# QualityMinds/cistgcn

Hardware: AMD Instinct MI355X
Metric: sequences/sec (fwd+bwd) H3.6M 22-joint 50->25 (higher is better)
Workload: dtype f32; 1 GPU; cistgcn64_b256_t50_v22; C=64, per_gpu_batch=256, global_batch=256, T_in=50, T_out=25, V=22, parallelism=dp1, graph=True, graph_branches=True, capture_kept=median, mixed_batches=False

## Files before the change

### cistgcn_amd/_lib.py

```python
import ctypes
import os
from ctypes import POINTER, c_double, c_float, c_int, c_int32, c_longlong, c_uint, c_ulonglong, c_void_p

HERE = os.path.dirname(os.path.abspath(__file__))
LIB_PATH = os.path.join(HERE, "libcistgcn_hip.so")

_handle = None
STAT_REPLICAS = 16
ALPHA_SLOTS = 64
_host_pointers_ok = False


class View4(ctypes.Structure):
    _fields_ = [("n", c_longlong * 4), ("s", c_longlong * 4)]


class NormAct(ctypes.Structure):
    _fields_ = [
        ("x", c_void_p), ("xv", View4),
        ("y", c_void_p), ("yv", View4),
        ("pre", c_void_p),
        ("add", c_void_p), ("av", View4),
        ("add_post", c_int),
        ("bn_mode", c_int),
# ... 101 lines not shown
                ("dx", c_void_p), ("dgamma", c_void_p), ("dbeta", c_void_p)]


class GatePath(ctypes.Structure):
    _fields_ = [("z", c_void_p), ("stats", c_void_p), ("stats_ld", c_longlong),
                ("bn2", TailBN), ("alpha2", c_void_p), ("Wl", c_void_p), ("bn3", TailBN), ("alpha3", c_void_p), ("W2", c_void_p),
                ("salt2", c_uint), ("salt3", c_uint), ("y", c_void_p), ("w", c_void_p), ("tap2", c_void_p), ("tap3", c_void_p),
                ("dw", c_void_p), ("dz", c_void_p), ("dstats", c_void_p), ("dWl", c_void_p), ("dW2", c_void_p),
                ("dgamma2", c_void_p), ("dbeta2", c_void_p), ("dalpha2", c_void_p), ("dgamma3", c_void_p), ("dbeta3", c_void_p), ("dalpha3", c_void_p),
                ("scratch", c_void_p), ("red", c_void_p)]


class GateHead(ctypes.Structure):
    _fields_ = [("B", c_int), ("C", c_int), ("S", c_int), ("train", c_int), ("n", c_int), ("pad", c_int),
                ("drop_p", c_float), ("pad2", c_int), ("seed", c_void_p), ("p", GatePath * 2)]


class CtxHeads(ctypes.Structure):
    _fields_ = [("B", c_int), ("P", c_int), ("C", c_int), ("train", c_int), ("x", c_void_p), ("xstats", c_void_p),
                ("w", c_void_p * 2), ("bn", TailBN * 2), ("alpha", c_void_p * 2),
                ("y", c_void_p * 2), ("arg", c_void_p), ("xsave", c_void_p), ("tap", c_void_p * 2),
                ("dy", c_void_p * 2), ("red", c_void_p), ("dx", c_void_p),
                ("dw", c_void_p * 2), ("dgamma", c_void_p * 2), ("dbeta", c_void_p * 2), ("dalpha", c_void_p * 2)]


class AttackStep(ctypes.Structure):
    _fields_ = [("B", c_int), ("T", c_int), ("V", c_int), ("mode", c_int), ("iterations", c_int), ("patience", c_int),
                ("epsilon", c_float), ("mu", c_float),
                ("x0", c_void_p), ("x", c_void_p), ("grad", c_void_p), ("g", c_void_p), ("mask", c_void_p), ("loss", c_void_p),
                ("best", c_void_p), ("stall", c_void_p), ("active", c_void_p), ("w", c_void_p), ("queries", c_void_p), ("n_active", c_void_p),
# ... 64 lines not shown
    "cg_collapse_sums_ws_floats": [c_int, c_int],
    "cg_fpn_conv_fwd": [POINTER(FpnConv), P],
    "cg_fpn_conv_bwd": [POINTER(FpnConv), P],
    "cg_fpn_conv_supported": [c_int, c_int, c_int, c_int, c_int],
    "cg_fpn_conv_ws_floats": [c_int, c_int, c_int, c_int],
    "cg_pointwise_maps_fwd": [POINTER(PwMaps), P],
    "cg_pointwise_maps_bwd": [POINTER(PwMaps), P],
    "cg_pointwise_maps_ws_floats": [c_int],
    "cg_block_input_fwd": [POINTER(BlockInput), P],
    "cg_block_input_bwd": [POINTER(BlockInput), P],
    "cg_block_input_supported": [c_int, c_int, c_int, c_int],
    "cg_gate_head_fwd": [POINTER(GateHead), P],
    "cg_gate_head_bwd": [POINTER(GateHead), P],
    "cg_gate_head_supported": [c_int, c_int, c_int],
    "cg_gate_head_scratch_floats": [c_int, c_int, c_int],
    "cg_context_heads_fwd": [POINTER(CtxHeads), P],
    "cg_context_heads_bwd": [POINTER(CtxHeads), P],
    "cg_context_heads_red_doubles": [c_int],
    "cg_map2adj_tail_fwd": [POINTER(AdjTail), c_int, c_int, P],
    "cg_map2adj_tail_bwd": [POINTER(AdjTail), c_int, c_int, P],
    "cg_map2adj_tail_ws_floats": [c_int],
    "cg_map2adj_tail_part_floats": [c_int, c_int, c_int],
    "cg_map2adj_tail_red_doubles": [c_int],
    "cg_augment_sequences": [P, P, P, P, P, P, P, P, P, P, c_int, c_int, c_int, c_int, P],
    "cg_map2adj_tail_geometry": [c_int, c_int, c_int, POINTER(c_int)],
    "cg_dstd_tail_geometry": [c_int, c_int, c_int, c_int, POINTER(c_int)],
    "cg_pointwise_maps_geometry": [c_int, c_int, c_int, c_int, POINTER(c_int), c_int, POINTER(c_int)],
    "cg_collapse_geometry": [c_int, c_int, c_int, c_int, c_int, c_int, POINTER(c_int)],
    "cg_fpn_conv_geometry": [c_int, c_int, c_int, c_int, c_int, POINTER(c_int)],
    "cg_stgcn_domain_geometry": [c_int, c_int, c_int, c_int, c_int, c_int, c_int, c_int, POINTER(c_int)],
# ... 47 lines not shown
```

### cistgcn_amd/models/CISTGCN/CISTGCN.py

```python
import torch
import torch.nn as nn

from ... import ops
from ..layers.SE import SELayer1d, SELayer2d


class Stage(nn.Module):

    def __init__(self, **slots):
        super().__init__()
        for k, m in slots.items():
            self.add_module(k.lstrip("s"), m)

    def __getitem__(self, i):
        return self._modules[str(i)]


def _conv(cin, cout, k=1, bias=False, **kw):
    return nn.Conv2d(cin, cout, k, bias=bias, **kw)


def _init_small(root, gain, convs):
    for m in root.modules():
        if isinstance(m, nn.Linear):
# ... 155 lines not shown
        p = arch.model_params
        self.clipping = p.clipping
        self.n_input, self.n_output, self.n_joints = p.input_n, p.output_n, p.joints
        self.n_txcnn_layers = p.n_txcnn_layers
        self.txc_kernel_size = [p.txc_kernel_size] * 2
        self.input_gcn, self.output_gcn = p.input_gcn, p.output_gcn
        self.reduction, self.hidden_dim = p.reduction, p.hidden_dim
        self.dropout = float(learn.dropout)
        self.in_ch = 10
        self.fused_domain = True
        self.staged = True
        self.fused_tail = True
        self.fused_adj = True
        self.fused_maps = True
        self.fused_defer = True
        self.stack_min_elements = 1 << 21
        widths = [self.in_ch] + list(p.input_gcn.model_complexity) + [self.in_ch]
        widths_o = [3] + list(p.output_gcn.model_complexity)
        T, V, To = self.n_input, self.n_joints, self.n_output

        self.st_gcnns = nn.ModuleList()
        self.txcnns = nn.ModuleList()
        self.se = nn.ModuleList()
        self.in_conv = nn.ModuleList()
        self.context_layer = nn.ModuleList()
        self.trans = nn.ModuleList()
        for i in range(len(widths) - 1):
            self.st_gcnns.append(DSTDBlock(widths[i], widths[i + 1], p.input_gcn.interpretable[i], T, V, self.reduction))
        self.context_layer = ContextLayer(self.hidden_dim, To, V, self.reduction)
        self.txcnns.append(FPN(T, To, p.txc_kernel_size))
# ... 160 lines not shown
            xa = list(ops.fanout(xn0, n_alias))
        x_stats, xn, x_dom = xa[0], xa[1], xa[2:4]
        k = 4
        x_maps = x_gates = None
        if stacked:
            x_maps, k = xa[4], 5
        if rows_gate:
            x_gates, k = xa[k], k + 1
        x_resmaps = []
        if res_groups:
            x_resmaps, k = xa[k:k + len(res_groups)], k + len(res_groups)
        x_res = xa[k:k + 2] if not has_res else None
        x_bres = xa[-1] if not has_bres else None
        if not fused_in:
            stats_s, stats_t = ops.fanout(ops.dstd_stats(x_stats), 2)
        gate_rows = None
        if gates:
            O = cs.out_channels
            w2 = ops.cat_channels([cs.weight.view(1, O, -1), ct.weight.view(1, O, -1)]).view(2 * O, cs.in_channels, xn.shape[2])
            if x_gates is not None:
                gate_rows = ops.collapse_rows(x_gates, w2)[0]
                items = []
            else:
                items = [(("och,bchw->bow", w2, xn, None, None, None), None)]
        else:
            items = [_rows_item(xn, cs, tr), _rows_item(xn, ct, tr)]
        if not stacked:
            for a in maps:
                items += [_pw_item(xn, a.time_compress[0], tr), _pw_item(xn, a.joint_compress[0], tr)]
        if res_groups is None:
            items += [_pw_item(xn, c, tr) for c in res_convs]
        o = _run_items(items) if items else []
        if gates:
            yg = gate_rows if gate_rows is not None else o.pop(0)[0]
            o = [(g.unsqueeze(2), None) for g in ops.split_channels(yg, (O, O))] + o
        towers_done, tower_tr = None, None
# ... 40 lines not shown
                o = o + ro
        gs, gt, tc = o[0], o[1], o[2:6]
        calls = [dict(x=gs, bn=m.conv_s[1], drop=True, prelu=m.conv_s[3]), dict(x=gt, bn=m.conv_t[1], drop=True, prelu=m.conv_t[3])]
        if towers_done is None:
            for i, a in enumerate(maps):
                calls += [dict(x=tc[2 * i], bn=a.time_compress[1], prelu=a.time_compress[2]),
                          dict(x=tc[2 * i + 1], bn=a.joint_compress[1], prelu=a.joint_compress[2])]
        k = 6
        n_tower_calls = len(calls) - 2
        if res_done is None:
            if has_res:
                calls += [dict(x=o[k + i], bn=d.residual[1]) for i, d in enumerate(doms)]
                k += 2
            if has_bres:
                calls.append(dict(x=o[k], bn=m.residual[1]))
        if towers_done is None:
            r = self._na_many(calls)
        else:
            r = self._na_many(calls[:2])
            self._site += 4
            r = r + towers_done + (self._na_many(calls[2 + n_tower_calls:]) if len(calls) > 2 + n_tower_calls else [])
        if res_done is not None:
            self._site += len(res_done)
            r = r + res_done
        gs, gt, t1 = r[0], r[1], r[2:6]
        res = r[6:8] if has_res else x_res
        bres = r[-1] if has_bres else x_bres
        items = [_cols_item(gs, m.conv_s[4], tr), _cols_item(gt, m.conv_t[4], tr)]
        rows3, cols3 = {}, {}
        for i, a in enumerate(maps):
            c3 = a.time_compress[3]
            x3 = t1[2 * i][0] if isinstance(t1[2 * i], tuple) else t1[2 * i]
            w3 = c3.weight.view(c3.out_channels, c3.in_channels, -1)
            if big and c3.bias is None and ops.collapse_rows_ok(x3, w3):
                y3, st3 = ops.collapse_rows(x3, w3, tr, transform=tower_tr[2 * i] if tower_tr else None)
                rows3[i] = (y3.unsqueeze(2), st3)
            else:
                assert tower_tr is None, "a deferred tower map needs its collapsing kernel"
                items.append(_rows_item(t1[2 * i], c3, tr))
            c4 = a.joint_compress[3]
            x4 = t1[2 * i + 1][0] if isinstance(t1[2 * i + 1], tuple) else t1[2 * i + 1]
            w4 = c4.weight.view(c4.out_channels, c4.in_channels, -1)
            if big and c4.bias is None and ops.collapse_cols_ok(x4, w4):
                y4, st4 = ops.collapse_cols(x4, w4, tr, transform=tower_tr[2 * i + 1] if tower_tr else None)
                cols3[i] = (y4.unsqueeze(3), st4)
            else:
                assert tower_tr is None, "a deferred tower map needs its collapsing kernel"
                items.append(_cols_item(t1[2 * i + 1], c4, tr))
        if tower_tr and self.act_trace is not None:
            tp_ = [b_ for a_ in maps for b_ in (a_.time_compress[2], a_.joint_compress[2])]
            for mod, tr_ in zip(tp_, tower_tr):
                self.act_trace[mod] = (tr_["tap"].detach(), None)
        o = _run_items(items)
        if rows3 or cols3:
            rest, o = o[2:], o[:2]
            for i in range(len(maps)):
                o.append(rows3[i] if i in rows3 else rest.pop(0))
                o.append(cols3[i] if i in cols3 else rest.pop(0))
        Cg = m.conv_s[4].out_channels
        gate_fused = (o[0][0].shape[1] == Cg and o[0][0].numel() == B * Cg and
                      ops.gate_head_ok(B, Cg, stats_s.shape[1], (m.conv_s[7], m.conv_t[7], m.map_s[3], m.map_t[3])))
        tower_calls = []
        for i, a in enumerate(maps):
            tower_calls += [dict(x=o[2 + 2 * i], bn=a.time_compress[4], drop=True), dict(x=o[3 + 2 * i], bn=a.joint_compress[4], drop=True)]
        if gate_fused:
            s2 = (self._site + 1, self._site + 2)
            self._site += 2
            r = [None, None] + self._na_many(tower_calls)
            s3 = (self._site + 1, self._site + 2)
            self._site += 2
            if self.drop_trace is not None:
                self.drop_trace[m.conv_s[5]], self.drop_trace[m.conv_t[5]], self.drop_trace[m.map_s[1]], self.drop_trace[m.map_t[1]] = s2[0], s2[1], s3[0], s3[1]
            taps = [] if self.act_trace is not None else None
            m.w1, m.w2 = ops.gate_head([o[0][0].view(B, Cg), o[1][0].view(B, Cg)], [stats_s, stats_t], [m.conv_s, m.conv_t], [m.map_s, m.map_t], tr,
                                       drop_p=self.dropout, salts=((s2[0], s3[0]), (s2[1], s3[1])), taps=taps)
            if taps is not None:
                self.act_trace[m.conv_s[7]], self.act_trace[m.map_s[3]] = (taps[0], None), (taps[1], None)
                self.act_trace[m.conv_t[7]], self.act_trace[m.map_t[3]] = (taps[2], None), (taps[3], None)
            items, g = [], None
        else:
            calls = [dict(x=o[0], bn=m.conv_s[5], drop=True, prelu=m.conv_s[7]), dict(x=o[1], bn=m.conv_t[5], drop=True, prelu=m.conv_t[7])]
            r = self._na_many(calls + tower_calls)
            hs = ops.cat_channels([r[0].view(B, -1), stats_s])
            ht = ops.cat_channels([r[1].view(B, -1), stats_t])
            items = [_lin_item(hs, m.map_s[0], tr), _lin_item(ht, m.map_t[0], tr)]
        for i, a in enumerate(maps):
            items += [_pw_item(r[2 + 2 * i], a.time_compress[6], False), _pw_item(r[3 + 2 * i], a.joint_compress[6], False)]
        o = _run_items(items)
        if gate_fused:
            o = [None, None] + o
        else:
            g = self._na_many([dict(x=o[0], bn=m.map_s[1], drop=True, prelu=m.map_s[3]), dict(x=o[1], bn=m.map_t[1], drop=True, prelu=m.map_t[3])])
        seeds = []
        for i, d in enumerate(doms):
            q, s = o[2 + 2 * i][0].view(B, T, V), o[3 + 2 * i][0].view(B, V, T)
            seeds.append((0 if d.domain == "space" else 1, s, q))
        if self.fused_adj and T <= 64 and V <= 64:
            if not gate_fused:
                o = _run_items([_lin_item(g[0], m.map_s[4], False), _lin_item(g[1], m.map_t[4], False)])
                m.w1, m.w2 = o[0][0], o[1][0]
            self._site += 2
            if self.drop_trace is not None:
                self.drop_trace[maps[0].expansor[1]], self.drop_trace[maps[1].expansor[1]] = self._site - 1, self._site
            taps = [] if self.act_trace is not None else None
            adj = ops.map2adj_tail(seeds, [a.expansor for a in maps], tr, drop_p=self.dropout, salts=(self._site - 1, self._site), taps=taps)
            adj = [(a, None) for a in adj]
            if taps is not None:
                for a, tap in zip(maps, taps):
                    self.act_trace[a.expansor[3]] = (tap, None)
        else:
            if T <= 64 and V <= 64:
                oo = ops.rank1_adj(seeds)
# ... 150 lines not shown
```

### cistgcn_amd/ops.py

```python
import ctypes
import os

import numpy as np
import torch

from . import _lib
from ._lib import NormAct, View4

_vp = ctypes.c_void_p


def _ptr(t):
    return _vp(t.data_ptr()) if t is not None else None


def _stream(t):
    if t.is_cuda:
        return _vp(torch.cuda.current_stream(t.device).cuda_stream)
    if not _lib._host_pointers_ok:
        raise RuntimeError("cistgcn_amd operators run on MI355X only: got a %s tensor (no CPU path exists)" % t.device)
    return None


def _chk(t, name="tensor"):
# ... 1935 lines not shown
        _lib.call("cg_gate_head_bwd", ctypes.byref(t), _stream(ts[0]))
        del keep
        return (None, None) + tuple(g if ctx.needs_input_grad[2 + k] else None for k, g in enumerate(grads))


def gate_head(zs, stats, convs, maps, train, drop_p=0.0, salts=((0, 0), (0, 0)), taps=None):
    n = len(zs)
    cfg = {"train": bool(train), "drop_p": float(drop_p), "salts": tuple((int(a), int(b)) for a, b in salts),
           "bn2": tuple(c[5] for c in convs), "bn3": tuple(m[1] for m in maps), "taps": taps}
    ts = []
    for z, st, c, m in zip(zs, stats, convs, maps):
        ts += [z, st, c[5].weight, c[5].bias, c[7].weight, m[0].weight, m[1].weight, m[1].bias, m[3].weight, m[4].weight]
    return list(_GateHead.apply(cfg, n, *ts))


def context_heads_ok(x, hidden):
    return x.dim() == 4 and x.shape[1] == 1 and x.is_contiguous() and hidden <= 64 and x.shape[2] * x.shape[3] <= 16384


class _ContextHeads(torch.autograd.Function):

    @staticmethod
    def _block(x, ts, bns, saves, train):
        B, _, H, W = x.shape
        t = _lib.CtxHeads()
        t.B, t.P, t.C, t.train = B, H * W, ts[0].numel(), 1 if train else 0
        t.x = x.data_ptr()
        for h in range(2):
            w, gamma, beta, alpha = ts[4 * h:4 * h + 4]
            t.w[h], t.alpha[h] = w.data_ptr(), alpha.data_ptr()
# ... 438 lines not shown
```

### include/cistgcn_hip.h

```cpp
#ifndef CISTGCN_HIP_H
#define CISTGCN_HIP_H
#include <stdint.h>
#ifdef __cplusplus
extern "C" {
#endif

#define CG_STAT_REPLICAS 16
#define CG_ALPHA_SLOTS 64

typedef struct CgView4 {
  long long n[4];
  long long s[4];
} CgView4;

int cg_contract(const float* A, const float* X, float* Y, const float* bias, double* stats, const int32_t* tables,
                int G, int M, int N, int K, int splitk, int a_kfast, int x_kfast,
                long long y_dense_numel, void* stream);

typedef struct CgContractDesc {
  const float* A; const float* X; float* Y; const float* bias; double* stats; const int32_t* tab;
  int G, M, N, K, splitk, kchunk , a_kfast, x_kfast;
  int accumulate;
  int x_vec;
  int stat_ch;
// ... 219 lines not shown
  float* dWl; float* dW2;
  float* dgamma2; float* dbeta2; float* dalpha2; float* dgamma3; float* dbeta3; float* dalpha3;
  float* scratch;
  double* red;
} CgGatePath;
typedef struct CgGateHead {
  int B, C, S, train, n, pad;
  float drop_p; int pad2; const unsigned long long* seed;
  CgGatePath p[2];
} CgGateHead;
int cg_gate_head_fwd(const CgGateHead* t, void* stream);
int cg_gate_head_bwd(const CgGateHead* t, void* stream);
int cg_gate_head_supported(int B, int C, int S);
long long cg_gate_head_scratch_floats(int B, int C, int S);

typedef struct CgCtxHeads {
  int B, P, C, train;
  const float* x;
  const double* xstats;
  const float* w[2]; CgTailBN bn[2]; const float* alpha[2];
  float* y[2];
  int32_t* arg;
  float* xsave;
  float* tap[2];
  const float* dy[2];
  double* red;
  float* dx;
  float* dw[2]; float* dgamma[2]; float* dbeta[2]; float* dalpha[2];
} CgCtxHeads;
int cg_context_heads_fwd(const CgCtxHeads* t, void* stream);
// ... 64 lines not shown
```

Baseline: 14750 sequences/sec.

## Fuse block mid-stage BN/PReLU/dropout/linear maps into batched multi-item kernel

Adds a block_mid HIP kernel family that, for up to six items per launch, applies batch norm from the producer's channel sums, PReLU and dropout, then a full linear map or a pointwise map, with matching two-kernel backward producing dx, dW, dgamma, dbeta and dalpha. The model's map stage routes through it instead of separate per-item launches and intermediate tensors. The aim is fewer launches and less global memory traffic for the normalized activations. In exchange it adds per-slice partial weight-gradient buffers and a second reduction pass, and it only runs for supported shapes.

```diff
diff --git a/cistgcn_amd/_lib.py b/cistgcn_amd/_lib.py
--- a/cistgcn_amd/_lib.py
+++ b/cistgcn_amd/_lib.py
@@ -139,6 +139,19 @@
 class GateHead(ctypes.Structure):
     _fields_ = [("B", c_int), ("C", c_int), ("S", c_int), ("train", c_int), ("n", c_int), ("pad", c_int),
                 ("drop_p", c_float), ("pad2", c_int), ("seed", c_void_p), ("p", GatePath * 2)]
+
+
+class MidItem(ctypes.Structure):
+    _fields_ = [("kind", c_int), ("C", c_int), ("L", c_int), ("O", c_int), ("sb_", c_int), ("ns_", c_int),
+                ("x", c_void_p), ("x_ld", c_longlong), ("bn", TailBN), ("stats_ld", c_longlong), ("alpha", c_void_p), ("W", c_void_p),
+                ("salt", c_uint), ("pad", c_int), ("y", c_void_p), ("tap", c_void_p),
+                ("dy", c_void_p), ("dx", c_void_p), ("dW", c_void_p), ("dgamma", c_void_p), ("dbeta", c_void_p), ("dalpha", c_void_p),
+                ("g", c_void_p), ("part", c_void_p), ("wpart", c_void_p)]
+
+
+class BlockMid(ctypes.Structure):
+    _fields_ = [("B", c_int), ("train", c_int), ("n", c_int), ("pad", c_int),
+                ("drop_p", c_float), ("pad2", c_int), ("seed", c_void_p), ("it", MidItem * 6)]
 
 
 class CtxHeads(ctypes.Structure):
@@ -233,6 +246,10 @@
     "cg_gate_head_bwd": [POINTER(GateHead), P],
     "cg_gate_head_supported": [c_int, c_int, c_int],
     "cg_gate_head_scratch_floats": [c_int, c_int, c_int],
+    "cg_block_mid_fwd": [POINTER(BlockMid), P],
+    "cg_block_mid_bwd": [POINTER(BlockMid), P],
+    "cg_block_mid_supported": [c_int, c_int, c_int, c_int, c_int],
+    "cg_block_mid_geometry": [c_int, c_int, c_int, c_int, c_int, POINTER(c_int)],
     "cg_context_heads_fwd": [POINTER(CtxHeads), P],
     "cg_context_heads_bwd": [POINTER(CtxHeads), P],
     "cg_context_heads_red_doubles": [c_int],
diff --git a/cistgcn_amd/csrc/block_mid.h b/cistgcn_amd/csrc/block_mid.h
--- /dev/null
+++ b/cistgcn_amd/csrc/block_mid.h
@@ -0,0 +1,27 @@
+#pragma once
+#include "dstd_tail.h"
+
+#define CG_MID_MAXN 6
+#define CG_MID_MAXD 64
+struct CgMidItem {
+  int kind, C, L, O;
+  int sb_, ns_;
+  const float* x; long long x_ld;
+  CgTailBN bn; long long stats_ld;
+  const float* alpha;
+  const float* W;
+  unsigned int salt; int pad;
+  float* y;
+  float* tap;
+  const float* dy;
+  float* dx;
+  float* dW; float* dgamma; float* dbeta; float* dalpha;
+  float* g;
+  double* part;
+  float* wpart;
+};
+struct CgBlockMid {
+  int B, train, n, pad;
+  float drop_p; int pad2; const unsigned long long* seed;
+  CgMidItem it[CG_MID_MAXN];
+};
diff --git a/cistgcn_amd/csrc/block_mid.hip b/cistgcn_amd/csrc/block_mid.hip
--- /dev/null
+++ b/cistgcn_amd/csrc/block_mid.hip
@@ -0,0 +1,402 @@
+#include "cg_common.h"
+#include "cg_phase.h"
+#include "block_mid.h"
+
+HIP_DYNAMIC_SHARED(unsigned char, cg_dyn_lds)
+
+#define CG_MID_THREADS 1024
+#define CG_MID_KSTEPS 4
+#define CG_MID_OSTEPS 8
+#define CG_MID_WAVES (CG_MID_THREADS / CG_WAVE)
+#define CG_MID_SB 8
+#define CG_MID_FULL_FLOATS 8192
+#define CG_MID_PW_FLOATS 4096
+
+static inline int cg_mid_pad4(int n) { return (n + 3) & ~3; }
+static inline int cg_mid_sb(int kind, int C, int L, int O) {
+  const int per = kind == 0 ? C * L : (C > O ? C : O) * L;
+  int sb = (kind == 0 ? CG_MID_FULL_FLOATS : CG_MID_PW_FLOATS) / per;
+  return sb < 1 ? 1 : (sb > CG_MID_SB ? CG_MID_SB : sb);
+}
+
+__device__ __forceinline__ void cg_mid_aff(const CgMidItem& it, int c, double cnt, int train, bool backward, bool owner, float* k) {
+  const CgTailBN& bn = it.bn;
+  const int C = it.C;
+  float mean, rstd;
+  if (backward) { mean = bn.save[c]; rstd = bn.save[C + c]; }
+  else if (train) {
+    double s1 = 0.0, s2 = 0.0;
+    for (int r = 0; r < CG_STAT_REPLICAS; ++r) { s1 += bn.stats[((long long)r * it.stats_ld + c) * 2]; s2 += bn.stats[((long long)r * it.stats_ld + c) * 2 + 1]; }
+    const double m = s1 / cnt;
+    double var = s2 / cnt - m * m;
+    if (var < 0.0) var = 0.0;
+    mean = (float)m;
+    rstd = (float)(1.0 / sqrt(var + (double)bn.eps));
+    if (owner && bn.running_mean) {
+      const double unb = cnt > 1.0 ? var * cnt / (cnt - 1.0) : var;
+      bn.running_mean[c] = (1.f - bn.momentum) * bn.running_mean[c] + bn.momentum * (float)m;
+      bn.running_var[c] = (1.f - bn.momentum) * bn.running_var[c] + bn.momentum * (float)unb;
+      if (c == 0 && bn.num_batches_tracked) *bn.num_batches_tracked += 1;
+    }
+  } else {
+    mean = bn.running_mean[c];
+    rstd = 1.0f / sqrtf(bn.running_var[c] + bn.eps);
+  }
+  if (!backward && owner) { bn.save[c] = mean; bn.save[C + c] = rstd; }
+  k[0] = mean; k[1] = rstd; k[2] = bn.gamma[c] * rstd; k[3] = bn.beta[c];
+}
+
+__device__ __forceinline__ float cg_mid_u(const CgBlockMid& t, const CgMidItem& it, const float (*sAff)[4], unsigned long long seed, bool drop,
+                                          int b, int r, int K, float& keep, float& xv) {
+  const int c = r / it.L;
+  xv = it.x[(long long)b * it.x_ld + r];
+  keep = drop ? cg_drop_scale(t.drop_p, seed, it.salt, (unsigned long long)b * K + r) : 1.f;
+  return ((xv - sAff[c][0]) * sAff[c][2] + sAff[c][3]) * keep;
+}
+
+__device__ __forceinline__ void cg_mid_stage_h(const CgBlockMid& t, const CgMidItem& it, const float (*sAff)[4], float* sH, int b0, int nb, bool tap) {
+  const int K = it.C * it.L;
+  const bool drop = t.train && t.drop_p > 0.f;
+  const unsigned long long seed = drop ? *t.seed : 0ull;
+  for (int e = threadIdx.x; e < it.sb_ * K; e += CG_MID_THREADS) {
+    const int b = e / K, r = e - b * K;
+    float h = 0.f;
+    if (b < nb) {
+      float keep, xv;
+      const float u = cg_mid_u(t, it, sAff, seed, drop, b0 + b, r, K, keep, xv);
+      h = it.alpha ? (u > 0.f ? u : it.alpha[0] * u) : u;
+      if (tap && it.tap) it.tap[(long long)(b0 + b) * K + r] = h;
+    }
+    sH[e] = h;
+  }
+}
+
+__global__ __launch_bounds__(CG_MID_THREADS) void cg_block_mid_fwd_kernel(CgBlockMid t) {
+  const CgMidItem& it = t.it[blockIdx.y];
+  if ((int)blockIdx.x >= it.ns_) return;
+  const int C = it.C, L = it.L, O = it.O, K = C * L, sb = it.sb_;
+  const int tid = threadIdx.x, lane = tid & (CG_WAVE - 1), wave = tid / CG_WAVE;
+  const int b0 = (int)blockIdx.x * sb, nb = min(sb, t.B - b0);
+  __shared__ float sAff[CG_MID_MAXD][4];
+  __shared__ double sRed[CG_MID_WAVES][4 * CG_MID_SB][4];
+  float* sH = reinterpret_cast<float*>(cg_dyn_lds);
+  float* sW = sH + ((sb * K + 3) & ~3);
+  const int OP = (O + 3) & ~3;
+  if (tid < C) cg_mid_aff(it, tid, (double)t.B * L, t.train, false, blockIdx.x == 0, sAff[tid]);
+  if (it.kind == 1)
+    for (int e = tid; e < C * OP; e += CG_MID_THREADS) { const int c = e / OP, o = e - c * OP; sW[e] = o < O ? it.W[o * C + c] : 0.f; }
+  __syncthreads();
+  cg_mid_stage_h(t, it, sAff, sH, b0, nb, true);
+  __syncthreads();
+  if (it.kind == 1) {
+    const int OG = OP >> 2, total = nb * OG * L;
+    for (int idx = tid; idx < total; idx += CG_MID_THREADS) {
+      const int l = idx % L, r = idx / L, og = r % OG, b = r / OG;
+      const float* h = sH + b * K + l;
+      const float* w = sW + 4 * og;
+      float acc[4] = {0.f, 0.f, 0.f, 0.f};
+      for (int c = 0; c < C; ++c) {
+        const float hv = h[c * L];
+        const float4 wv = *reinterpret_cast<const float4*>(w + c * OP);
+        acc[0] = fmaf(wv.x, hv, acc[0]); acc[1] = fmaf(wv.y, hv, acc[1]); acc[2] = fmaf(wv.z, hv, acc[2]); acc[3] = fmaf(wv.w, hv, acc[3]);
+      }
+#pragma unroll
+      for (int j = 0; j < 4; ++j)
+        if (4 * og + j < O) it.y[((long long)(b0 + b) * O + 4 * og + j) * L + l] = acc[j];
+    }
+    return;
+  }
+  const int OG = (O + 3) >> 2, iters = (OG + CG_MID_WAVES - 1) / CG_MID_WAVES;
+  for (int i = 0; i < iters; ++i) {
+    const int og = i * CG_MID_WAVES + wave;
+    float acc[4][CG_MID_SB];
+#pragma unroll
+    for (int j = 0; j < 4; ++j)
+#pragma unroll
+      for (int b = 0; b < CG_MID_SB; ++b) acc[j][b] = 0.f;
+    if (og < OG) {
+      const float* w[4];
+#pragma unroll
+      for (int j = 0; j < 4; ++j) w[j] = it.W + (long long)min(4 * og + j, O - 1) * K;
+      for (int k0 = lane; k0 < K; k0 += CG_MID_KSTEPS * CG_WAVE) {
+        float wv[CG_MID_KSTEPS][4];
+#pragma unroll
+        for (int s = 0; s < CG_MID_KSTEPS; ++s)
+#pragma unroll
+          for (int j = 0; j < 4; ++j) wv[s][j] = k0 + s * CG_WAVE < K ? w[j][k0 + s * CG_WAVE] : 0.f;
+#pragma unroll
+        for (int s = 0; s < CG_MID_KSTEPS; ++s) {
+          const int k = k0 + s * CG_WAVE;
+          if (k < K) {
+#pragma unroll
+            for (int b = 0; b < CG_MID_SB; ++b)
+              if (b < sb) {
+                const float hv = sH[b * K + k];
+#pragma unroll
+                for (int j = 0; j < 4; ++j) acc[j][b] = fmaf(wv[s][j], hv, acc[j][b]);
+              }
+          }
+        }
+      }
+    }
+#pragma unroll
+    for (int j = 0; j < 4; ++j)
+#pragma unroll
+      for (int b = 0; b < CG_MID_SB; ++b) {
+        const double v = cg_row16_sum((double)acc[j][b]);
+        if ((lane & 15) == 0) sRed[wave][j * CG_MID_SB + b][lane >> 4] = v;
+      }
+    __syncthreads();
+    if (tid < CG_MID_WAVES * 4 * CG_MID_SB) {
+      const int w2 = tid / (4 * CG_MID_SB), q = tid - w2 * (4 * CG_MID_SB), j = q / CG_MID_SB, b = q - j * CG_MID_SB;
+      const int o = 4 * (i * CG_MID_WAVES + w2) + j;
+      if (o < O && b < nb) it.y[(long long)(b0 + b) * O + o] = (float)((sRed[w2][q][0] + sRed[w2][q][1]) + (sRed[w2][q][2] + sRed[w2][q][3]));
+    }
+    __syncthreads();
+  }
+}
+
+__global__ __launch_bounds__(CG_MID_THREADS) void cg_block_mid_bwd1_kernel(CgBlockMid t) {
+  const CgMidItem& it = t.it[blockIdx.y];
+  if ((int)blockIdx.x >= it.ns_) return;
+  const int C = it.C, L = it.L, O = it.O, K = C * L, sb = it.sb_;
+  const int tid = threadIdx.x, lane = tid & (CG_WAVE - 1), wave = tid / CG_WAVE;
+  const int slice = (int)blockIdx.x, b0 = slice * sb, nb = min(sb, t.B - b0);
+  __shared__ float sAff[CG_MID_MAXD][4];
+  __shared__ double sRedD[CG_MID_WAVES];
+  const int HK = (sb * K + 3) & ~3;
+  float* sH = reinterpret_cast<float*>(cg_dyn_lds);
+  float* sG = sH + HK;
+  float* sDy = sG + HK;
+  const int CP = (C + 3) & ~3;
+  float* sW = sDy + (it.kind == 0 ? O * CG_MID_SB : ((sb * O * L + 3) & ~3));
+  if (tid < C) cg_mid_aff(it, tid, 0.0, t.train, true, false, sAff[tid]);
+  if (it.kind == 0) {
+    for (int e = tid; e < O * CG_MID_SB; e += CG_MID_THREADS) {
+      const int o = e / CG_MID_SB, b = e - o * CG_MID_SB;
+      sDy[e] = b < nb ? it.dy[(long long)(b0 + b) * O + o] : 0.f;
+    }
+  } else {
+    for (int e = tid; e < O * CP; e += CG_MID_THREADS) { const int o = e / CP, c = e - o * CP; sW[e] = c < C ? it.W[o * C + c] : 0.f; }
+    for (int e = tid; e < nb * O * L; e += CG_MID_THREADS) sDy[e] = it.dy[(long long)b0 * O * L + e];
+  }
+  __syncthreads();
+  cg_mid_stage_h(t, it, sAff, sH, b0, nb, false);
+  __syncthreads();
+  if (it.kind == 0) {
+    float* wp = it.wpart + (long long)slice * O * K;
+    for (int k = tid; k < K; k += CG_MID_THREADS) {
+      float hv[CG_MID_SB], dh[CG_MID_SB];
+#pragma unroll
+      for (int b = 0; b < CG_MID_SB; ++b) { hv[b] = b < sb ? sH[b * K + k] : 0.f; dh[b] = 0.f; }
+      for (int o0 = 0; o0 < O; o0 += CG_MID_OSTEPS) {
+        float wv[CG_MID_OSTEPS];
+#pragma unroll
+        for (int s = 0; s < CG_MID_OSTEPS; ++s) wv[s] = o0 + s < O ? it.W[(long long)(o0 + s) * K + k] : 0.f;
+#pragma unroll
+        for (int s = 0; s < CG_MID_OSTEPS; ++s) {
+          const int o = o0 + s;
+          if (o < O) {
+            const float4 d0 = *reinterpret_cast<const float4*>(sDy + o * CG_MID_SB), d1 = *reinterpret_cast<const float4*>(sDy + o * CG_MID_SB + 4);
+            const float d[CG_MID_SB] = {d0.x, d0.y, d0.z, d0.w, d1.x, d1.y, d1.z, d1.w};
+            float a = 0.f;
+#pragma unroll
+            for (int b = 0; b < CG_MID_SB; ++b) { dh[b] = fmaf(wv[s], d[b], dh[b]); a = fmaf(d[b], hv[b], a); }
+            wp[(long long)o * K + k] = a;
+          }
+        }
+      }
+#pragma unroll
+      for (int b = 0; b < CG_MID_SB; ++b) if (b < sb) sG[b * K + k] = dh[b];
+    }
+  } else {
+    float* wp = it.wpart + (long long)slice * O * C;
+    const int OG = (O + 3) >> 2;
+    for (int e = tid; e < OG * C; e += CG_MID_THREADS) {
+      const int og = e / C, c = e - og * C;
+      int oo[4];
+#pragma unroll
+      for (int j = 0; j < 4; ++j) oo[j] = min(4 * og + j, O - 1);
+      float a[4] = {0.f, 0.f, 0.f, 0.f};
+      for (int b = 0; b < nb; ++b) {
+        const float* h = sH + b * K + c * L;
+        const float* d = sDy + b * O * L;
+        float ab[4] = {0.f, 0.f, 0.f, 0.f};
+        for (int l = 0; l < L; ++l) {
+          const float hv = h[l];
+#pragma unroll
+          for (int j = 0; j < 4; ++j) ab[j] = fmaf(d[oo[j] * L + l], hv, ab[j]);
+        }
+#pragma unroll
+        for (int j = 0; j < 4; ++j) a[j] += ab[j];
+      }
+#pragma unroll
+      for (int j = 0; j < 4; ++j) if (4 * og + j < O) wp[(4 * og + j) * C + c] = a[j];
+    }
+    const int CG = CP >> 2, total = nb * CG * L;
+    for (int idx = tid; idx < total; idx += CG_MID_THREADS) {
+      const int l = idx % L, r = idx / L, cg = r % CG, b = r / CG;
+      const float* d = sDy + b * O * L + l;
+      float acc[4] = {0.f, 0.f, 0.f, 0.f};
+      for (int o = 0; o < O; ++o) {
+        const float dv = d[o * L];
+        const float4 wv = *reinterpret_cast<const float4*>(sW + o * CP + 4 * cg);
+        acc[0] = fmaf(wv.x, dv, acc[0]); acc[1] = fmaf(wv.y, dv, acc[1]); acc[2] = fmaf(wv.z, dv, acc[2]); acc[3] = fmaf(wv.w, dv, acc[3]);
+      }
+#pragma unroll
+      for (int j = 0; j < 4; ++j) if (4 * cg + j < C) sG[b * K + (4 * cg + j) * L + l] = acc[j];
+    }
+  }
+  __syncthreads();
+  const bool drop = t.train && t.drop_p > 0.f;
+  const unsigned long long seed = drop ? *t.seed : 0ull;
+  const float alpha = it.alpha ? it.alpha[0] : 1.f;
+  double SA = 0.0;
+  for (int e = tid; e < nb * K; e += CG_MID_THREADS) {
+    const int b = e / K, r = e - b * K;
+    float keep, xv;
+    const float u = cg_mid_u(t, it, sAff, seed, drop, b0 + b, r, K, keep, xv);
+    const float dh = sG[e];
+    const bool neg = it.alpha && !(u > 0.f);
+    if (neg) SA += (double)dh * (double)u;
+    const float g = (neg ? alpha * dh : dh) * keep;
+    sG[e] = g;
+    it.g[(long long)(b0 + b) * K + r] = g;
+  }
+  __syncthreads();
+  double* part = it.part + (long long)slice * (2 * C + 1);
+  for (int c = wave; c < C; c += CG_MID_WAVES) {
+    double s1 = 0.0, s2 = 0.0;
+    const float mean = sAff[c][0], rstd = sAff[c][1];
+    for (int i = lane; i < nb * L; i += CG_WAVE) {
+      const int b = i / L, l = i - b * L;
+      const double v = (double)sG[b * K + c * L + l];
+      s1 += v;
+      s2 += v * (double)((it.x[(long long)(b0 + b) * it.x_ld + c * L + l] - mean) * rstd);
+    }
+    s1 = cg_wave_sum(s1); s2 = cg_wave_sum(s2);
+    if (lane == 0) { part[c] = s1; part[C + c] = s2; }
+  }
+  SA = cg_block_sum(SA, sRedD);
+  if (tid == 0) part[2 * C] = SA;
+}
+
+__global__ __launch_bounds__(CG_MID_THREADS) void cg_block_mid_bwd2_kernel(CgBlockMid t) {
+  const CgMidItem& it = t.it[blockIdx.y];
+  if ((int)blockIdx.x >= it.ns_) return;
+  const int C = it.C, L = it.L, O = it.O, K = C * L, sb = it.sb_, ns = it.ns_, nv = 2 * C + 1;
+  const int tid = threadIdx.x, lane = tid & (CG_WAVE - 1), wave = tid / CG_WAVE;
+  const int slice = (int)blockIdx.x, b0 = slice * sb, nb = min(sb, t.B - b0);
+  __shared__ float sAff[CG_MID_MAXD][4];
+  __shared__ double sP[CG_MID_WAVES][2 * CG_MID_MAXD + 1];
+  __shared__ float sM[CG_MID_MAXD][2];
+  if (tid < C) cg_mid_aff(it, tid, 0.0, t.train, true, false, sAff[tid]);
+  for (int v = lane; v < nv; v += CG_WAVE) {
+    double s = 0.0;
+    for (int sl = wave; sl < ns; sl += CG_MID_WAVES) s += it.part[(long long)sl * nv + v];
+    sP[wave][v] = s;
+  }
+  __syncthreads();
+  if (tid < C) {
+    double S1 = 0.0, S2 = 0.0;
+    for (int w = 0; w < CG_MID_WAVES; ++w) { S1 += sP[w][tid]; S2 += sP[w][C + tid]; }
+    const double cnt = (double)t.B * L;
+    sM[tid][0] = t.train ? (float)(S1 / cnt) : 0.f; sM[tid][1] = t.train ? (float)(S2 / cnt) : 0.f;
+    if (slice == 0) { it.dgamma[tid] = (float)S2; it.dbeta[tid] = (float)S1; }
+  }
+  if (tid == 0 && slice == 0 && it.dalpha) {
+    double SA = 0.0;
+    for (int w = 0; w < CG_MID_WAVES; ++w) SA += sP[w][2 * C];
+    it.dalpha[0] = (float)SA;
+  }
+  __syncthreads();
+  for (int e = tid; e < nb * K; e += CG_MID_THREADS) {
+    const int b = e / K, r = e - b * K, c = r / L;
+    const long long idx = (long long)(b0 + b) * K + r;
+    const float xv = it.x[(long long)(b0 + b) * it.x_ld + r];
+    it.dx[idx] = sAff[c][2] * (it.g[idx] - sM[c][0] - (xv - sAff[c][0]) * sAff[c][1] * sM[c][1]);
+  }
+  const long long NW = (long long)O * (it.kind == 0 ? K : C), chunk = (NW + ns - 1) / ns;
+  const long long e1 = min(NW, (slice + 1) * chunk);
+  for (long long e = slice * chunk + tid; e < e1; e += CG_MID_THREADS) {
+    double a = 0.0;
+    for (int sl = 0; sl < ns; ++sl) a += (double)it.wpart[sl * NW + e];
+    it.dW[e] = (float)a;
+  }
+}
+
+static size_t cg_mid_lds_fwd(int kind, int C, int L, int O) {
+  const int sb = cg_mid_sb(kind, C, L, O);
+  return ((size_t)cg_mid_pad4(sb * C * L) + (kind == 1 ? (size_t)C * cg_mid_pad4(O) : 0)) * sizeof(float);
+}
+static size_t cg_mid_lds_bwd(int kind, int C, int L, int O) {
+  const int sb = cg_mid_sb(kind, C, L, O);
+  size_t f = (size_t)2 * cg_mid_pad4(sb * C * L);
+  f += kind == 0 ? (size_t)O * CG_MID_SB : (size_t)cg_mid_pad4(sb * O * L) + (size_t)O * cg_mid_pad4(C);
+  return f * sizeof(float);
+}
+
+extern "C" int cg_block_mid_supported(int B, int kind, int C, int L, int O) {
+  if (B <= 0 || kind < 0 || kind > 1 || C <= 0 || L <= 0 || O <= 0 || C > CG_MID_MAXD || L > CG_MID_MAXD || O > CG_MID_MAXD) return 0;
+  const int sb = cg_mid_sb(kind, C, L, O);
+  const long long ns = ((long long)B + sb - 1) / sb;
+  return (ns <= 65535 && ns * O * C * (kind == 0 ? L : 1) < (1ll << 31)) ? 1 : 0;
+}
+
+extern "C" int cg_block_mid_geometry(int B, int kind, int C, int L, int O, int* out) {
+  if (!out || !cg_block_mid_supported(B, kind, C, L, O)) return CG_ESHAPE;
+  const int sb = cg_mid_sb(kind, C, L, O), ns = (B + sb - 1) / sb;
+  out[0] = sb; out[1] = ns;
+  out[2] = (int)cg_mid_lds_fwd(kind, C, L, O); out[3] = (int)cg_mid_lds_bwd(kind, C, L, O);
+  out[4] = ns * (2 * C + 1);
+  out[5] = ns * O * C * (kind == 0 ? L : 1);
+  out[6] = kind == 0 ? (((O + 3) >> 2) + CG_MID_WAVES - 1) / CG_MID_WAVES : 0;
+  out[7] = kind == 0 ? (C * L + CG_MID_THREADS - 1) / CG_MID_THREADS : 0;
+  return CG_OK;
+}
+
+static int cg_mid_prepare(const CgBlockMid* t, bool bwd, CgBlockMid& a, int& slices, size_t& lds) {
+  if (!t || t->n < 1 || t->n > CG_MID_MAXN || t->B <= 0) return CG_EARG;
+  if (t->drop_p < 0.f || t->drop_p >= 1.f) return CG_EARG;
+  if (t->train && t->drop_p > 0.f && !t->seed) return CG_EARG;
+  a = *t;
+  slices = 0; lds = 0;
+  for (int i = 0; i < t->n; ++i) {
+    CgMidItem& p = a.it[i];
+    if (!cg_block_mid_supported(t->B, p.kind, p.C, p.L, p.O)) return CG_ESHAPE;
+    if (t->train && (long long)t->B * p.L < 2) return CG_ESHAPE;
+    if (!p.x || p.x_ld < (long long)p.C * p.L || !p.W || !p.bn.gamma || !p.bn.beta || !p.bn.save) return CG_EARG;
+    if (!bwd && (!p.y || (t->train ? (!p.bn.stats || p.stats_ld < p.C) : (!p.bn.running_mean || !p.bn.running_var)))) return CG_EARG;
+    if (bwd && (!p.dy || !p.dx || !p.dW || !p.dgamma || !p.dbeta || (p.alpha && !p.dalpha) || !p.g || !p.part || !p.wpart)) return CG_EARG;
+    p.sb_ = cg_mid_sb(p.kind, p.C, p.L, p.O);
+    p.ns_ = (t->B + p.sb_ - 1) / p.sb_;
+    if (p.ns_ > slices) slices = p.ns_;
+    const size_t l = bwd ? cg_mid_lds_bwd(p.kind, p.C, p.L, p.O) : cg_mid_lds_fwd(p.kind, p.C, p.L, p.O);
+    if (l > lds) lds = l;
+  }
+  return CG_OK;
+}
+
+extern "C" int cg_block_mid_fwd(const CgBlockMid* t, void* stream_) {
+  CgBlockMid a;
+  int slices; size_t lds;
+  int st = cg_mid_prepare(t, false, a, slices, lds);
+  if (st != CG_OK) return st;
+  if (lds > CG_LDS_DEFAULT && cg_lds_limit((const void*)cg_block_mid_fwd_kernel, lds) != hipSuccess) return CG_ESHAPE;
+  hipLaunchKernelGGL(cg_block_mid_fwd_kernel, dim3((unsigned)slices, (unsigned)a.n), dim3(CG_MID_THREADS), lds, (hipStream_t)stream_, a);
+  return cg_launch_status();
+}
+
+extern "C" int cg_block_mid_bwd(const CgBlockMid* t, void* stream_) {
+  CgBlockMid a;
+  int slices; size_t lds;
+  int st = cg_mid_prepare(t, true, a, slices, lds);
+  if (st != CG_OK) return st;
+  if (lds > CG_LDS_DEFAULT && cg_lds_limit((const void*)cg_block_mid_bwd1_kernel, lds) != hipSuccess) return CG_ESHAPE;
+  const dim3 grid((unsigned)slices, (unsigned)a.n), block(CG_MID_THREADS);
+  hipLaunchKernelGGL(cg_block_mid_bwd1_kernel, grid, block, lds, (hipStream_t)stream_, a);
+  st = cg_launch_status();
+  if (st != CG_OK) return st;
+  hipLaunchKernelGGL(cg_block_mid_bwd2_kernel, grid, block, 0, (hipStream_t)stream_, a);
+  return cg_launch_status();
+}
diff --git a/cistgcn_amd/models/CISTGCN/CISTGCN.py b/cistgcn_amd/models/CISTGCN/CISTGCN.py
--- a/cistgcn_amd/models/CISTGCN/CISTGCN.py
+++ b/cistgcn_amd/models/CISTGCN/CISTGCN.py
@@ -193,6 +193,7 @@
         self.fused_adj = True
         self.fused_maps = True
         self.fused_defer = True
+        self.fused_mid = True
         self.stack_min_elements = 1 << 21
         widths = [self.in_ch] + list(p.input_gcn.model_complexity) + [self.in_ch]
         widths_o = [3] + list(p.output_gcn.model_complexity)
@@ -383,12 +384,19 @@
         x_bres = xa[-1] if not has_bres else None
         if not fused_in:
             stats_s, stats_t = ops.fanout(ops.dstd_stats(x_stats), 2)
-        gate_rows = None
+        gate_rows = gate_sums = None
+        adj_fused = self.fused_adj and T <= 64 and V <= 64
+        mid_on = self.fused_mid and big and adj_fused
+        g4s, g4t = m.conv_s[4], m.conv_t[4]
+        mid_g = (mid_on and gates and x_gates is not None and g4s.bias is None and g4t.bias is None
+                 and tuple(g4s.kernel_size) == (1, V) and tuple(g4t.kernel_size) == (1, V) and g4s.out_channels == g4t.out_channels
+                 and ops.gate_head_ok(B, g4s.out_channels, 2 + 2 * T, (m.conv_s[7], m.conv_t[7], m.map_s[3], m.map_t[3]))
+                 and ops.block_mid_ok(B, [(0, cs.out_channels, V, g4s.out_channels, m.conv_s[3]), (0, cs.out_channels, V, g4t.out_channels, m.conv_t[3])]))
         if gates:
             O = cs.out_channels
             w2 = ops.cat_channels([cs.weight.view(1, O, -1), ct.weight.view(1, O, -1)]).view(2 * O, cs.in_channels, xn.shape[2])
             if x_gates is not None:
-                gate_rows = ops.collapse_rows(x_gates, w2)[0]
+                gate_rows, gate_sums = ops.collapse_rows(x_gates, w2, mid_g and tr)
                 items = []
             else:
                 items = [(("och,bchw->bow", w2, xn, None, None, None), None)]
@@ -459,10 +467,16 @@
                 k += 2
             if has_bres:
                 calls.append(dict(x=o[k], bn=m.residual[1]))
+        mid_x = mid_salts = None
+        if mid_g:
+            mid_x, mid_salts = [gs[0].squeeze(2), gt[0].squeeze(2)], (self._site + 1, self._site + 2)
+            self._site += 2
+            if self.drop_trace is not None:
+                self.drop_trace[m.conv_s[1]], self.drop_trace[m.conv_t[1]] = mid_salts
         if towers_done is None:
-            r = self._na_many(calls)
-        else:
-            r = self._na_many(calls[:2])
+            r = [None, None] + (self._na_many(calls[2:]) if len(calls) > 2 else []) if mid_g else self._na_many(calls)
+        else:
+            r = [None, None] if mid_g else self._na_many(calls[:2])
             self._site += 4
             r = r + towers_done + (self._na_many(calls[2 + n_tower_calls:]) if len(calls) > 2 + n_tower_calls else [])
         if res_done is not None:
@@ -471,7 +485,7 @@
         gs, gt, t1 = r[0], r[1], r[2:6]
         res = r[6:8] if has_res else x_res
         bres = r[-1] if has_bres else x_bres
-        items = [_cols_item(gs, m.conv_s[4], tr), _cols_item(gt, m.conv_t[4], tr)]
+        items = [] if mid_g else [_cols_item(gs, m.conv_s[4], tr), _cols_item(gt, m.conv_t[4], tr)]
         rows3, cols3 = {}, {}
         for i, a in enumerate(maps):
             c3 = a.time_compress[3]
@@ -496,26 +510,57 @@
             tp_ = [b_ for a_ in maps for b_ in (a_.time_compress[2], a_.joint_compress[2])]
             for mod, tr_ in zip(tp_, tower_tr):
                 self.act_trace[mod] = (tr_["tap"].detach(), None)
-        o = _run_items(items)
+        o = ([None, None] if mid_g else []) + (_run_items(items) if items else [])
         if rows3 or cols3:
             rest, o = o[2:], o[:2]
             for i in range(len(maps)):
                 o.append(rows3[i] if i in rows3 else rest.pop(0))
                 o.append(cols3[i] if i in cols3 else rest.pop(0))
         Cg = m.conv_s[4].out_channels
-        gate_fused = (o[0][0].shape[1] == Cg and o[0][0].numel() == B * Cg and
-                      ops.gate_head_ok(B, Cg, stats_s.shape[1], (m.conv_s[7], m.conv_t[7], m.map_s[3], m.map_t[3])))
+        gate_fused = mid_g or (o[0][0].shape[1] == Cg and o[0][0].numel() == B * Cg and
+                               ops.gate_head_ok(B, Cg, stats_s.shape[1], (m.conv_s[7], m.conv_t[7], m.map_s[3], m.map_t[3])))
         tower_calls = []
         for i, a in enumerate(maps):
             tower_calls += [dict(x=o[2 + 2 * i], bn=a.time_compress[4], drop=True), dict(x=o[3 + 2 * i], bn=a.joint_compress[4], drop=True)]
+        tower_mid = [(a.time_compress, a.joint_compress)[k] for a in maps for k in (0, 1)]
+        mid_t = (mid_on and gate_fused and len(rows3) == len(maps) and len(cols3) == len(maps) and all(c[6].bias is None for c in tower_mid)
+                 and ops.block_mid_ok(B, [(1, o[2 + k][0].shape[1], o[2 + k][0].numel() // (B * o[2 + k][0].shape[1]), c[6].out_channels, None)
+                                          for k, c in enumerate(tower_mid)]))
         if gate_fused:
             s2 = (self._site + 1, self._site + 2)
             self._site += 2
-            r = [None, None] + self._na_many(tower_calls)
+            if mid_t:
+                tower_salts = tuple(self._site + 1 + k for k in range(len(tower_mid)))
+                self._site += len(tower_mid)
+                if self.drop_trace is not None:
+                    for c, salt in zip(tower_mid, tower_salts):
+                        self.drop_trace[c[4]] = salt
+                r = [None] * (2 + len(tower_mid))
+            else:
+                r = [None, None] + self._na_many(tower_calls)
             s3 = (self._site + 1, self._site + 2)
             self._site += 2
             if self.drop_trace is not None:
                 self.drop_trace[m.conv_s[5]], self.drop_trace[m.conv_t[5]], self.drop_trace[m.map_s[1]], self.drop_trace[m.map_t[1]] = s2[0], s2[1], s3[0], s3[1]
+            mid_out = []
+            if mid_g or mid_t:
+                mitems = []
+                if mid_g:
+                    for i, cv in enumerate((m.conv_s, m.conv_t)):
+                        mitems.append(dict(kind=0, x=mid_x[i], bn=cv[1], prelu=cv[3], weight=cv[4].weight.view(Cg, -1, V), salt=mid_salts[i],
+                                           stats=(gate_sums, i * mid_x[i].shape[1], 2 * mid_x[i].shape[1]) if tr else None))
+                if mid_t:
+                    for k, c in enumerate(tower_mid):
+                        y, st = o[2 + k]
+                        mitems.append(dict(kind=1, x=y.view(B, y.shape[1], -1), bn=c[4], prelu=None, weight=c[6].weight.view(c[6].out_channels, y.shape[1]),
+                                           salt=tower_salts[k], stats=(st, 0, y.shape[1]) if tr else None))
+                mtaps = [] if self.act_trace is not None else None
+                mid_out = ops.block_mid(mitems, tr, drop_p=self.dropout, taps=mtaps)
+                if mid_g:
+                    o[0], o[1] = (mid_out[0], None), (mid_out[1], None)
+                    mid_out = mid_out[2:]
+                    if mtaps is not None:
+                        self.act_trace[m.conv_s[3]], self.act_trace[m.conv_t[3]] = (mtaps[0].unsqueeze(2), None), (mtaps[1].unsqueeze(2), None)
             taps = [] if self.act_trace is not None else None
             m.w1, m.w2 = ops.gate_head([o[0][0].view(B, Cg), o[1][0].view(B, Cg)], [stats_s, stats_t], [m.conv_s, m.conv_t], [m.map_s, m.map_t], tr,
                                        drop_p=self.dropout, salts=((s2[0], s3[0]), (s2[1], s3[1])), taps=taps)
@@ -529,9 +574,12 @@
             hs = ops.cat_channels([r[0].view(B, -1), stats_s])
             ht = ops.cat_channels([r[1].view(B, -1), stats_t])
             items = [_lin_item(hs, m.map_s[0], tr), _lin_item(ht, m.map_t[0], tr)]
-        for i, a in enumerate(maps):
-            items += [_pw_item(r[2 + 2 * i], a.time_compress[6], False), _pw_item(r[3 + 2 * i], a.joint_compress[6], False)]
-        o = _run_items(items)
+        if mid_t:
+            o = [(y, None) for y in mid_out]
+        else:
+            for i, a in enumerate(maps):
+                items += [_pw_item(r[2 + 2 * i], a.time_compress[6], False), _pw_item(r[3 + 2 * i], a.joint_compress[6], False)]
+            o = _run_items(items)
         if gate_fused:
             o = [None, None] + o
         else:
@@ -540,7 +588,7 @@
         for i, d in enumerate(doms):
             q, s = o[2 + 2 * i][0].view(B, T, V), o[3 + 2 * i][0].view(B, V, T)
             seeds.append((0 if d.domain == "space" else 1, s, q))
-        if self.fused_adj and T <= 64 and V <= 64:
+        if adj_fused:
             if not gate_fused:
                 o = _run_items([_lin_item(g[0], m.map_s[4], False), _lin_item(g[1], m.map_t[4], False)])
                 m.w1, m.w2 = o[0][0], o[1][0]
diff --git a/cistgcn_amd/ops.py b/cistgcn_amd/ops.py
--- a/cistgcn_amd/ops.py
+++ b/cistgcn_amd/ops.py
@@ -1973,6 +1973,127 @@
     return list(_GateHead.apply(cfg, n, *ts))
 
 
+def _mid_geometry(B, kind, C, L, O):
+    out = (ctypes.c_int * 8)()
+    _lib.check(_lib.lib().cg_block_mid_geometry(B, kind, C, L, O, out), "cg_block_mid_geometry")
+    return list(out)
+
+
+def block_mid_ok(B, items):
+    return 1 <= len(items) <= 6 and all(bool(_lib.lib().cg_block_mid_supported(B, k, C, L, O)) and (p is None or p.weight.numel() == 1)
+                                        for k, C, L, O, p in items)
+
+
+class _BlockMid(torch.autograd.Function):
+
+    @staticmethod
+    def _block(cfg, ts, saves, train, dev):
+        items = cfg["items"]
+        t = _lib.BlockMid()
+        t.B, t.train, t.n = ts[0].shape[0], 1 if train else 0, len(items)
+        p = float(cfg.get("drop_p", 0.0)) if train else 0.0
+        t.drop_p = p
+        if p > 0.0:
+            t.seed = seed_state(dev).data_ptr()
+        for i, it in enumerate(items):
+            x, _, _, a, w = ts[5 * i:5 * i + 5]
+            q = t.it[i]
+            q.kind, q.C, q.L, q.O = it["kind"], x.shape[1], x.shape[2], w.shape[0]
+            q.x, q.x_ld = x.data_ptr(), x.stride(0)
+            _tail_bn(q.bn, it["bn"], None, saves[i], train)
+            st = it.get("stats")
+            if train and st is not None:
+                q.bn.stats, q.stats_ld = st[0].data_ptr() + 16 * st[1], st[2]
+            q.alpha, q.W, q.salt = _ptr(a), w.data_ptr(), it["salt"]
+        return t, p
+
+    @staticmethod
+    def forward(ctx, cfg, *ts):
+        ctx.set_materialize_grads(False)
+        items = cfg["items"]
+        dev, f32, train = ts[0].device, torch.float32, bool(cfg["train"])
+        B = ts[0].shape[0]
+        ts = list(ts)
+        for i, it in enumerate(items):
+            x, w = ts[5 * i], ts[5 * i + 4]
+            _chk(x)
+            C, L = x.shape[1], x.shape[2]
+            if x.dim() != 3 or (L > 1 and x.stride(2) != 1) or (C > 1 and x.stride(1) != L) or x.stride(0) < C * L:
+                raise ValueError("block_mid expects (B,C,L) inputs with dense samples")
+            if w.numel() != w.shape[0] * C * (L if it["kind"] == 0 else 1):
+                raise ValueError("block_mid: weight %s does not fit input %s" % (tuple(w.shape), tuple(x.shape)))
+            if not w.is_contiguous():
+                ts[5 * i + 4] = _copy(w)
+            if train and it.get("stats") is None:
+                raise ValueError("block_mid needs the producer's channel sums in train mode")
+            if train and B * L < 2:
+                raise ValueError("Expected more than 1 value per channel when training, got input size %s" % (tuple(x.shape),))
+        saves = [torch.empty(2, ts[5 * i].shape[1], dtype=f32, device=dev) for i in range(len(items))]
+        t, p = _BlockMid._block(cfg, ts, saves, train, dev)
+        taps = cfg.get("taps")
+        ys = []
+        for i, it in enumerate(items):
+            x, w = ts[5 * i], ts[5 * i + 4]
+            ys.append(torch.empty((B, w.shape[0]) if it["kind"] == 0 else (B, w.shape[0], x.shape[2]), dtype=f32, device=dev))
+            t.it[i].y = ys[-1].data_ptr()
+            if taps is not None:
+                taps.append(torch.empty(x.shape, dtype=f32, device=dev) if ts[5 * i + 3] is not None else None)
+                t.it[i].tap = _ptr(taps[-1])
+        _lib.call("cg_block_mid_fwd", ctypes.byref(t), _stream(ts[0]))
+        ctx.cfg, ctx.p = cfg, p
+        ctx.seed_epoch = seed_epoch(dev) if p > 0.0 else None
+        ctx.has_alpha = [ts[5 * i + 3] is not None for i in range(len(items))]
+        ctx.save_for_backward(*[v for v in ts if v is not None], *saves)
+        return tuple(ys)
+
+    @staticmethod
+    def backward(ctx, *dys):
+        cfg = ctx.cfg
+        items = cfg["items"]
+        n = len(items)
+        sv = list(ctx.saved_tensors)
+        saves = sv[len(sv) - n:]
+        ts = []
+        for i in range(n):
+            ts += [sv.pop(0), sv.pop(0), sv.pop(0), sv.pop(0) if ctx.has_alpha[i] else None, sv.pop(0)]
+        dev, f32, train = ts[0].device, torch.float32, bool(cfg["train"])
+        _check_seed_epoch(ctx, dev, "block_mid")
+        B = ts[0].shape[0]
+        t, _ = _BlockMid._block(cfg, ts, saves, train, dev)
+        keep, grads = [], []
+        for i, it in enumerate(items):
+            x, _, _, a, w = ts[5 * i:5 * i + 5]
+            C, L, O = x.shape[1], x.shape[2], w.shape[0]
+            d = dys[i]
+            if d is None:
+                d = _zeros(B * O * (1 if it["kind"] == 0 else L), dev)[0]
+            d = d if d.is_contiguous() else _copy(d)
+            geo = _mid_geometry(B, it["kind"], C, L, O)
+            dx = torch.empty(B, C, L, dtype=f32, device=dev)
+            dw = torch.empty(w.shape, dtype=f32, device=dev)
+            small = torch.empty(3, C, dtype=f32, device=dev)
+            g = torch.empty(B * C * L, dtype=f32, device=dev)
+            part = torch.empty(geo[4], dtype=torch.float64, device=dev)
+            wpart = torch.empty(geo[5], dtype=f32, device=dev)
+            q = t.it[i]
+            q.dy, q.dx, q.dW, q.g, q.part, q.wpart = d.data_ptr(), dx.data_ptr(), dw.data_ptr(), g.data_ptr(), part.data_ptr(), wpart.data_ptr()
+            q.dgamma, q.dbeta, q.dalpha = small[0].data_ptr(), small[1].data_ptr(), small[2].data_ptr() if a is not None else None
+            keep += [d, g, part, wpart]
+            grads += [dx, small[0], small[1], small[2, :1].reshape(a.shape) if a is not None else None, dw]
+        _lib.call("cg_block_mid_bwd", ctypes.byref(t), _stream(ts[0]))
+        del keep
+        return (None,) + tuple(g if (g is not None and ctx.needs_input_grad[1 + k]) else None for k, g in enumerate(grads))
+
+
+def block_mid(items, train, drop_p=0.0, taps=None):
+    cfg = {"train": bool(train), "drop_p": float(drop_p), "taps": taps,
+           "items": tuple({"kind": int(it["kind"]), "bn": it["bn"], "salt": int(it["salt"]), "stats": it.get("stats")} for it in items)}
+    ts = []
+    for it in items:
+        ts += [it["x"], it["bn"].weight, it["bn"].bias, it["prelu"].weight if it.get("prelu") is not None else None, it["weight"]]
+    return list(_BlockMid.apply(cfg, *ts))
+
+
 def context_heads_ok(x, hidden):
     return x.dim() == 4 and x.shape[1] == 1 and x.is_contiguous() and hidden <= 64 and x.shape[2] * x.shape[3] <= 16384
 
diff --git a/include/cistgcn_hip.h b/include/cistgcn_hip.h
--- a/include/cistgcn_hip.h
+++ b/include/cistgcn_hip.h
@@ -257,6 +257,33 @@
 int cg_gate_head_supported(int B, int C, int S);
 long long cg_gate_head_scratch_floats(int B, int C, int S);
 
+typedef struct CgMidItem {
+  int kind, C, L, O;
+  int sb_, ns_;
+  const float* x; long long x_ld;
+  CgTailBN bn; long long stats_ld;
+  const float* alpha;
+  const float* W;
+  unsigned int salt; int pad;
+  float* y;
+  float* tap;
+  const float* dy;
+  float* dx;
+  float* dW; float* dgamma; float* dbeta; float* dalpha;
+  float* g;
+  double* part;
+  float* wpart;
+} CgMidItem;
+typedef struct CgBlockMid {
+  int B, train, n, pad;
+  float drop_p; int pad2; const unsigned long long* seed;
+  CgMidItem it[6];
+} CgBlockMid;
+int cg_block_mid_fwd(const CgBlockMid* t, void* stream);
+int cg_block_mid_bwd(const CgBlockMid* t, void* stream);
+int cg_block_mid_supported(int B, int kind, int C, int L, int O);
+int cg_block_mid_geometry(int B, int kind, int C, int L, int O, int* out);
+
 typedef struct CgCtxHeads {
   int B, P, C, train;
   const float* x;
```

Result: faster. 14950 sequences/sec (median of 6 runs) (+1.3%).
